# olof3/QuantumOptimalControl.jl

Measured on AMD Instinct MI355X. Metric: GRAPE gradient evals/sec (dim N, T slices, B seeds) @ 1/2/4/8 GPU, higher is better.
Workload: dtype f64

## Files before the change

quantumoptimalcontrol.jl_amd/csrc/qoc_blkseg.hpp:

```cpp
#pragma once
#include "qoc_blku.hpp"

namespace qoc {

struct BlksegParams {
  double rad[3];
  double mur[3], mui[3];
  double theta_cap;
  int S;
  int L;
  int UPW;
  int RB;
  const double* u;
  double* u_copy;
  double* u_copy2;
  double* J2;
  cx<double>* coef2;
  double* dJdu;
  unsigned long long* terms;
  unsigned int* done;
  double* best;
  long long seed_offset;
  double* best_res;
  double* best_out;
// ... 231 lines not shown
        for (int kk = 0; kk < NB; ++kk) {
          double sr = 0.0, si = 0.0;
#pragma unroll
          for (int q = 0; q < NB; ++q) {
            sr = fma(Rr[i * NB + q], xr_[q * NB + kk], fma(-Ri[i * NB + q], xi_[q * NB + kk], sr));
            si = fma(Rr[i * NB + q], xi_[q * NB + kk], fma(Ri[i * NB + q], xr_[q * NB + kk], si));
          }
          tr[kk] = sr;
          ti[kk] = si;
        }
#pragma unroll
        for (int kk = 0; kk < NB; ++kk) {
          Rr[i * NB + kk] = tr[kk];
          Ri[i * NB + kk] = ti[kk];
        }
      }
#pragma unroll
      for (int kk = 0; kk < NB; ++kk) {
        double tr[NB], ti[NB];
#pragma unroll
        for (int i = 0; i < NB; ++i) {
          double sr = Rr[i * NB + kk], si = Ri[i * NB + kk];
#pragma unroll
          for (int q = 0; q < NB; ++q) {
            sr = fma(xr_[i * NB + q], Lr[q * NB + kk], fma(-xi_[i * NB + q], Li[q * NB + kk], sr));
            si = fma(xr_[i * NB + q], Li[q * NB + kk], fma(xi_[i * NB + q], Lr[q * NB + kk], si));
          }
          tr[i] = sr;
          ti[i] = si;
        }
#pragma unroll
        for (int i = 0; i < NB; ++i) {
          Lr[i * NB + kk] = tr[i];
          Li[i * NB + kk] = ti[i];
          if constexpr (MACC) {
            Mr[i * NB + kk] = fma(invf[n + 1], tr[i], Mr[i * NB + kk]);
            Mi[i * NB + kk] = fma(invf[n + 1], ti[i], Mi[i * NB + kk]);
          }
        }
      }
      if constexpr (!MACC) seg_trace<NB>(gen, Lr, Li, invf[n + 1], m1r, m1i, m2r, m2i, acc1, acc2);
    }
  }
  if constexpr (MACC) seg_trace<NB>(gen, Mr, Mi, 1.0, m1r, m1i, m2r, m2i, acc1, acc2);
}

struct Sk2 {
  double d0, d1, r, q;
};
__device__ __forceinline__ Sk2 sk2_of(const double2 (&e)[4]) { return Sk2{e[0].y, e[3].y, e[1].x, e[1].y}; }

template <int K = BLKSEG_KMAX>
__device__ __forceinline__ void sk2_phase(double d0, double d1, double& ct, double& st) {
  constexpr BlksegTrig T = blkseg_trig();
  const double t = 0.5 * (d0 + d1), t2 = t * t;
  ct = T.c[K];
  st = T.s[K];
#pragma unroll
  for (int k = K - 1; k >= 0; --k) {
    ct = fma(ct, t2, T.c[k]);
    st = fma(st, t2, T.s[k]);
  }
  st *= t;
}
template <int K = BLKSEG_KMAX>
__device__ __forceinline__ void sk2_z(const Sk2& g0, const double* rec, double& zr, double& zi) {
  double ct, st;
  sk2_phase<K>(g0.d0, g0.d1, ct, st);
  const double2 ph = *reinterpret_cast<const double2*>(rec);
  zr = ph.x * ct - ph.y * st;
  zi = fma(ph.x, st, ph.y * ct);
}
template <int K = BLKSEG_KMAX, bool EX = false>
__device__ __forceinline__ void sk2_form(const Sk2 (&g)[3], double2 ph, double2 u, Sk2& ah, double (&ur)[4],
                                         double (&ui)[4], double* ex = nullptr) {
  constexpr BlksegTrig T = blkseg_trig();
  ah.d0 = fma(u.y, g[2].d0, fma(u.x, g[1].d0, g[0].d0));
  ah.d1 = fma(u.y, g[2].d1, fma(u.x, g[1].d1, g[0].d1));
  ah.r = fma(u.y, g[2].r, fma(u.x, g[1].r, g[0].r));
  ah.q = fma(u.y, g[2].q, fma(u.x, g[1].q, g[0].q));
  const double a = 0.5 * (ah.d0 - ah.d1);
  const double w = fma(a, a, fma(ah.r, ah.r, ah.q * ah.q));
  double cw = T.c[K], sw = T.s[K], s3 = EX ? T.d[K] : 0.0, ct, st;
#pragma unroll
  for (int k = K - 1; k >= 0; --k) {
    cw = fma(cw, w, T.c[k]);
    sw = fma(sw, w, T.s[k]);
    if constexpr (EX) s3 = fma(s3, w, T.d[k]);
  }
  sk2_phase<K>(ah.d0, ah.d1, ct, st);
  const double zr = ph.x * ct - ph.y * st, zi = fma(ph.x, st, ph.y * ct);
  const double cr = zr * cw, ci = zi * cw, sr = zr * sw, si = zi * sw;
  if constexpr (EX) {
    ex[0] = cw;
    ex[1] = sw;
    ex[2] = s3;
    ex[3] = zr;
    ex[4] = zi;
  }
  ur[0] = fma(-si, a, cr);
  ui[0] = fma(sr, a, ci);
  ur[3] = fma(si, a, cr);
  ui[3] = fma(-sr, a, ci);
  ur[1] = fma(sr, ah.r, -si * ah.q);
  ui[1] = fma(sr, ah.q, si * ah.r);
  ur[2] = fma(-sr, ah.r, -si * ah.q);
  ui[2] = fma(sr, ah.q, -si * ah.r);
}
template <int K = BLKSEG_KMAX, bool EX = false>
__device__ __forceinline__ void sk2_form_v(const Sk2 (&g)[3], double2 u, double a0, Sk2& ah, double (&v)[4],
                                           double zr = 1.0, double zi = 0.0, double* ex = nullptr) {
  constexpr BlksegTrig T = blkseg_trig();
  ah.d0 = g[0].d0;
  ah.d1 = g[0].d1;
  ah.r = fma(u.y, g[2].r, fma(u.x, g[1].r, g[0].r));
  ah.q = fma(u.y, g[2].q, fma(u.x, g[1].q, g[0].q));
  const double w = fma(a0, a0, fma(ah.r, ah.r, ah.q * ah.q));
  double cw = T.c[K], sw = T.s[K], s3 = EX ? T.d[K] : 0.0;
#pragma unroll
  for (int k = K - 1; k >= 0; --k) {
    cw = fma(cw, w, T.c[k]);
    sw = fma(sw, w, T.s[k]);
    if constexpr (EX) s3 = fma(s3, w, T.d[k]);
  }
  if constexpr (EX) {
    ex[0] = cw;
    ex[1] = sw;
    ex[2] = s3;
    ex[3] = zr;
    ex[4] = zi;
  }
  v[0] = cw;
  v[1] = sw * a0;
  v[2] = sw * ah.r;
  v[3] = sw * ah.q;
}
__device__ __forceinline__ void sk2_expand(const double (&v)[4], double (&mr)[4], double (&mi)[4]) {
  mr[0] = v[0];
  mi[0] = v[1];
  mr[1] = v[2];
  mi[1] = v[3];
  mr[2] = -v[2];
  mi[2] = v[3];
  mr[3] = v[0];
  mi[3] = -v[1];
}
__device__ __forceinline__ void sk2_vmul(const double (&v)[4], const double (&p)[4], double (&t)[4]) {
  t[0] = fma(v[0], p[0], fma(-v[1], p[1], fma(-v[2], p[2], -v[3] * p[3])));
  t[1] = fma(v[0], p[1], fma(v[1], p[0], fma(v[2], p[3], -v[3] * p[2])));
  t[2] = fma(v[0], p[2], fma(-v[1], p[3], fma(v[2], p[0], v[3] * p[1])));
  t[3] = fma(v[0], p[3], fma(v[1], p[2], fma(-v[2], p[1], v[3] * p[0])));
}

__device__ __forceinline__ void sk2_rx(double (&Rr)[4], double (&Ri)[4], const Sk2& x) {
#pragma unroll
  for (int i = 0; i < 2; ++i) {
    const double p0r = Rr[2 * i], p0i = Ri[2 * i], p1r = Rr[2 * i + 1], p1i = Ri[2 * i + 1];
    Rr[2 * i] = fma(-p0i, x.d0, fma(-p1r, x.r, -p1i * x.q));
    Ri[2 * i] = fma(p0r, x.d0, fma(p1r, x.q, -p1i * x.r));
    Rr[2 * i + 1] = fma(p0r, x.r, fma(-p0i, x.q, -p1i * x.d1));
    Ri[2 * i + 1] = fma(p0r, x.q, fma(p0i, x.r, p1r * x.d1));
  }
}
__device__ __forceinline__ void sk2_xlr(double (&Lr)[4], double (&Li)[4], const double (&Rr)[4], const double (&Ri)[4],
                                        const Sk2& x) {
#pragma unroll
  for (int k = 0; k < 2; ++k) {
    const double c0r = Lr[k], c0i = Li[k], c1r = Lr[2 + k], c1i = Li[2 + k];
    Lr[k] = fma(-x.d0, c0i, fma(x.r, c1r, fma(-x.q, c1i, Rr[k])));
    Li[k] = fma(x.d0, c0r, fma(x.r, c1i, fma(x.q, c1r, Ri[k])));
    Lr[2 + k] = fma(-x.r, c0r, fma(-x.q, c0i, fma(-x.d1, c1i, Rr[2 + k])));
    Li[2 + k] = fma(-x.r, c0i, fma(x.q, c0r, fma(x.d1, c1r, Ri[2 + k])));
  }
}
template <int ORD>
__device__ __forceinline__ void sk2_contract(const Sk2& x, const Sk2& e1, const Sk2& e2, double (&Lr)[4],
                                             double (&Li)[4], double& acc1, double& acc2) {
  constexpr double invf[6] = {1.0, 1.0, 0.5, 1.0 / 6, 1.0 / 24, 1.0 / 120};
  double Mr[4], Mi[4], Rr[4], Ri[4];
#pragma unroll
  for (int e = 0; e < 4; ++e) {
    Mr[e] = Rr[e] = Lr[e];
    Mi[e] = Ri[e] = Li[e];
  }
#pragma unroll
  for (int n = 1; n < ORD; ++n) {
    sk2_rx(Rr, Ri, x);
    sk2_xlr(Lr, Li, Rr, Ri, x);
#pragma unroll
    for (int e = 0; e < 4; ++e) {
      Mr[e] = fma(invf[n + 1], Lr[e], Mr[e]);
      Mi[e] = fma(invf[n + 1], Li[e], Mi[e]);
    }
  }
  const double dr = Mr[2] - Mr[1], di = Mi[2] + Mi[1];
  acc1 = fma(-e1.d0, Mi[0], fma(-e1.d1, Mi[3], fma(e1.r, dr, -e1.q * di)));
  acc2 = fma(-e2.d0, Mi[0], fma(-e2.d1, Mi[3], fma(e2.r, dr, -e2.q * di)));
}

template <int ORD, bool CX = false>
__device__ __forceinline__ void sk2_contract_pauli(const Sk2& x, const double (&a1)[4], const double (&a2)[4],
                                                   const double (&Kr)[4], const double (&Ki)[4], double& acc1,
                                                   double& acc2, double x0c = 0.0, double x3c = 0.0,
                                                   double x02c = 0.0) {
  static_assert(ORD >= 1 && ORD <= 3, "Pauli form for orders 1..3");
  const double k0i = Ki[0] + Ki[3], k1i = Ki[1] + Ki[2], k2i = Kr[1] - Kr[2], k3i = Ki[0] - Ki[3];
  if constexpr (CX) {
    double m1, m2;
    if constexpr (ORD == 1) {
      m1 = k1i;
      m2 = k2i;
    } else {
      const double k0r = Kr[0] + Kr[3], k1r = Kr[1] + Kr[2], k2r = Ki[2] - Ki[1];
      const double x1 = x.q, x2 = x.r;
      if constexpr (ORD == 2) {
        m1 = fma(x0c, k1r, fma(k0r, x1, k1i));
        m2 = fma(x0c, k2r, fma(k0r, x2, k2i));
      } else {
        const double di = fma(x3c, k3i, fma(x2, k2i, x1 * k1i));
        const double w = fma(x3c, x3c, fma(x2, x2, x1 * x1));
        const double al1 = fma(-0.5, x02c, fma(-1.0 / 6.0, w, 1.0));
        const double c = fma(-x0c, k0i, fma(-1.0 / 3.0, di, k0r));
        m1 = fma(al1, k1i, fma(x0c, k1r, c * x1));
        m2 = fma(al1, k2i, fma(x0c, k2r, c * x2));
      }
    }
    acc1 = fma(a1[2], m2, a1[1] * m1);
    acc2 = fma(a2[2], m2, a2[1] * m1);
    return;
  }
  double m0, m1, m2, m3;
  if constexpr (ORD == 1) {
    m0 = k0i;
    m1 = k1i;
    m2 = k2i;
    m3 = k3i;
  } else {
    const double k0r = Kr[0] + Kr[3], k1r = Kr[1] + Kr[2], k2r = Ki[2] - Ki[1], k3r = Kr[0] - Kr[3];
    const double x0 = CX ? x0c : 0.5 * (x.d0 + x.d1), x1 = x.q, x2 = x.r, x3 = CX ? x3c : 0.5 * (x.d0 - x.d1);
    const double dr = fma(x3, k3r, fma(x2, k2r, x1 * k1r)), di = fma(x3, k3i, fma(x2, k2i, x1 * k1i));
    if constexpr (ORD == 2) {
      m0 = fma(x0, k0r, k0i + dr);
      m1 = fma(x0, k1r, fma(k0r, x1, k1i));
      m2 = fma(x0, k2r, fma(k0r, x2, k2i));
      m3 = fma(x0, k3r, fma(k0r, x3, k3i));
    } else {
      const double w = fma(x3, x3, fma(x2, x2, x1 * x1)), x02 = CX ? x02c : x0 * x0;
      const double al0 = fma(-0.5, x02 + w, 1.0), al1 = fma(-0.5, x02, fma(-1.0 / 6.0, w, 1.0));
      m0 = fma(al0, k0i, fma(x0, k0r - di, dr));
      const double c = fma(-x0, k0i, fma(-1.0 / 3.0, di, k0r));
      m1 = fma(al1, k1i, fma(x0, k1r, c * x1));
      m2 = fma(al1, k2i, fma(x0, k2r, c * x2));
      m3 = fma(al1, k3i, fma(x0, k3r, c * x3));
    }
  }
  acc1 = fma(a1[3], m3, fma(a1[2], m2, fma(a1[1], m1, a1[0] * m0)));
  acc2 = fma(a2[3], m3, fma(a2[2], m2, fma(a2[1], m1, a2[0] * m0)));
}
__device__ __forceinline__ void sk2_pauli2(const Sk2& e, double (&a)[4]) {
  a[0] = -0.5 * (e.d0 + e.d1);
  a[1] = -0.5 * (2.0 * e.q);
  a[2] = -0.5 * (2.0 * e.r);
  a[3] = -0.5 * (e.d0 - e.d1);
}

template <bool CX = false>
__device__ __forceinline__ void sk2_contract_exact(const Sk2& x, const double (&a1)[4], const double (&a2)[4],
                                                   const double (&Kr)[4], const double (&Ki)[4], const double (&ex)[5],
                                                   double& acc1, double& acc2, double x3c = 0.0) {
  const double cw = ex[0], sw = ex[1], s3 = ex[2], zr = ex[3], zi = ex[4];
  const double k0i = Ki[0] + Ki[3], k1i = Ki[1] + Ki[2], k2i = Kr[1] - Kr[2], k3i = Ki[0] - Ki[3];
  const double k0r = Kr[0] + Kr[3], k1r = Kr[1] + Kr[2], k2r = Ki[2] - Ki[1], k3r = Kr[0] - Kr[3];
  const double x1 = x.q, x2 = x.r, x3 = CX ? x3c : 0.5 * (x.d0 - x.d1);
  const double dr = fma(x3, k3r, fma(x2, k2r, x1 * k1r)), di = fma(x3, k3i, fma(x2, k2i, x1 * k1i));
  const double cr = -fma(sw, k0i, s3 * dr), ci = fma(sw, k0r, -s3 * di);
  const double m1 = fma(zr, fma(sw, k1i, ci * x1), zi * fma(sw, k1r, cr * x1));
  const double m2 = fma(zr, fma(sw, k2i, ci * x2), zi * fma(sw, k2r, cr * x2));
  if constexpr (CX) {
    acc1 = fma(a1[2], m2, a1[1] * m1);
    acc2 = fma(a2[2], m2, a2[1] * m1);
  } else {
    const double n0r = fma(cw, k0r, -sw * di), n0i = fma(cw, k0i, sw * dr);
    const double m0 = fma(zr, n0i, zi * n0r);
    const double m3 = fma(zr, fma(sw, k3i, ci * x3), zi * fma(sw, k3r, cr * x3));
    acc1 = fma(a1[3], m3, fma(a1[2], m2, fma(a1[1], m1, a1[0] * m0)));
    acc2 = fma(a2[3], m3, fma(a2[2], m2, fma(a2[1], m1, a2[0] * m0)));
  }
}

template <int NB>
__device__ __forceinline__ void seg_rx(double (&Rr)[NB * NB], double (&Ri)[NB * NB], const double (&xr_)[NB * NB],
                                       const double (&xi_)[NB * NB]) {
#pragma unroll
  for (int i = 0; i < NB; ++i) {
    double tr[NB], ti[NB];
#pragma unroll
    for (int kk = 0; kk < NB; ++kk) {
      double sr = 0.0, si = 0.0;
#pragma unroll
      for (int q = 0; q < NB; ++q) {
        sr = fma(Rr[i * NB + q], xr_[q * NB + kk], fma(-Ri[i * NB + q], xi_[q * NB + kk], sr));
        si = fma(Rr[i * NB + q], xi_[q * NB + kk], fma(Ri[i * NB + q], xr_[q * NB + kk], si));
      }
      tr[kk] = sr;
      ti[kk] = si;
    }
#pragma unroll
    for (int kk = 0; kk < NB; ++kk) {
      Rr[i * NB + kk] = tr[kk];
      Ri[i * NB + kk] = ti[kk];
    }
  }
}
template <int NB>
__device__ __forceinline__ void seg_xlr(double (&Lr)[NB * NB], double (&Li)[NB * NB], const double (&Rr)[NB * NB],
                                        const double (&Ri)[NB * NB], const double (&xr_)[NB * NB],
                                        const double (&xi_)[NB * NB]) {
#pragma unroll
  for (int kk = 0; kk < NB; ++kk) {
    double tr[NB], ti[NB];
#pragma unroll
    for (int i = 0; i < NB; ++i) {
      double sr = Rr[i * NB + kk], si = Ri[i * NB + kk];
#pragma unroll
      for (int q = 0; q < NB; ++q) {
        sr = fma(xr_[i * NB + q], Lr[q * NB + kk], fma(-xi_[i * NB + q], Li[q * NB + kk], sr));
        si = fma(xr_[i * NB + q], Li[q * NB + kk], fma(xi_[i * NB + q], Lr[q * NB + kk], si));
      }
      tr[i] = sr;
      ti[i] = si;
    }
#pragma unroll
    for (int i = 0; i < NB; ++i) {
      Lr[i * NB + kk] = tr[i];
      Li[i * NB + kk] = ti[i];
    }
  }
}
template <int NB, typename GENF>
__device__ __forceinline__ void seg_contract_exact(GENF&& genf, const double (&xr_)[NB * NB], const double (&xi_)[NB * NB],
                                                   double (&Lr)[NB * NB], double (&Li)[NB * NB], int nex, double er,
                                                   double ei, double m1r, double m1i, double m2r, double m2i,
                                                   double& acc1, double& acc2) {
  constexpr int E = NB * NB;
  double Rr[E], Ri[E];
#pragma unroll
  for (int e = 0; e < E; ++e) {
    const double vr = Lr[e], vi = Li[e];
    Lr[e] = Rr[e] = er * vr - ei * vi;
    Li[e] = Ri[e] = fma(er, vi, ei * vr);
  }
  acc1 = acc2 = 0.0;
  seg_trace<NB>(genf(), Lr, Li, 1.0, m1r, m1i, m2r, m2i, acc1, acc2);
  double f = 1.0;
#pragma unroll 1
  for (int n = 1; n < nex; ++n) {
    seg_rx<NB>(Rr, Ri, xr_, xi_);
    seg_xlr<NB>(Lr, Li, Rr, Ri, xr_, xi_);
    f /= (double)(n + 1);
    seg_trace<NB>(genf(), Lr, Li, f, m1r, m1i, m2r, m2i, acc1, acc2);
  }
}

__device__ __forceinline__ double block_max(double v, double* scratch) {
  for (int off = 32; off > 0; off >>= 1) v = fmax(v, __shfl_xor(v, off));
  const int w = threadIdx.x >> 6, l = threadIdx.x & 63;
  __syncthreads();
  if (l == 0) scratch[w] = v;
  __syncthreads();
  double s = scratch[0];
  const int nw = (blockDim.x + 63) >> 6;
  for (int i = 1; i < nw; ++i) s = fmax(s, scratch[i]);
  __syncthreads();
  return s;
}

__device__ __forceinline__ void wave_lds_sync() {
  __builtin_amdgcn_fence(__ATOMIC_RELEASE, "wavefront");
  __builtin_amdgcn_wave_barrier();
  __builtin_amdgcn_fence(__ATOMIC_ACQUIRE, "wavefront");
}
// ... 813 lines not shown
        }
        seg_mm<NB, false, false>(qr, qi, dr, di, tr, ti);
#pragma unroll
        for (int i = 0; i < NB; ++i)
#pragma unroll
          for (int j = 0; j < NB; ++j) {
            double sr = 0.0, si = 0.0;
#pragma unroll
            for (int q = 0; q < NB; ++q) {
              sr = fma(tr[i * NB + q], qr[j * NB + q], fma(ti[i * NB + q], qi[j * NB + q], sr));
              si = fma(ti[i * NB + q], qr[j * NB + q], fma(-tr[i * NB + q], qi[j * NB + q], si));
            }
            if constexpr (MODE == BLKSEG_FWD) dseg_at(i * NB + j) = make_double2(sr, si);
            else dl_at(i * NB + j) = make_double2(sr, si);
          }
        __builtin_amdgcn_sched_barrier(0);
        const double f = 2.0 * sp.pen_mu;
#pragma unroll
        for (int i = 0; i < NB; ++i)
#pragma unroll
          for (int j = 0; j < NB; ++j) {
            double sr = 0.0, si = 0.0;
#pragma unroll
            for (int q = 0; q < NB; ++q) {
              sr = fma(dr[i * NB + q], Hr[q * NB + j], fma(-di[i * NB + q], Hi[q * NB + j], sr));
              si = fma(dr[i * NB + q], Hi[q * NB + j], fma(di[i * NB + q], Hr[q * NB + j], si));
            }
            hr[i * NB + j] = fma(f, sr, hr[i * NB + j]);
            hi[i * NB + j] = fma(f, si, hi[i * NB + j]);
          }
        __builtin_amdgcn_sched_barrier(0);
      }
    }
    seg_mm<NB, false, false>(qr, qi, hr, hi, tr, ti);
    seg_mm<NB, false, true>(tr, ti, qr, qi, Gr, Gi);
  }

  if (!early) publish();
  BK_T(t2e);
  BK_ADD(2, t2e - t2);
  if constexpr (MODE == BLKSEG_FWD) {
    if (sact)
#pragma unroll
      for (int e = 0; e < E; ++e) gseg_at(e) = make_double2(Gr[e], Gi[e]);
    if (sp.terms && tid == 0) atomicAdd(sp.terms + b % TERM_SLOTS, (unsigned long long)Nt * ((unsigned long long)P << J));
    return;
  }
  }
  BK_T(t3);
  const double mu1r = sp.mur[1], mu1i = sp.mui[1], mu2r = sp.mur[2], mu2i = sp.mui[2];
  const double pen2 = PEN ? 2.0 * sp.pen_mu : 0.0;
  auto pen_step = [&](const double (&ur)[E], const double (&ui)[E]) {
    seg_pen_step<NB>(pm, pen2, slot + (size_t)opaque(s) * E * nblk + beta, nblk, ur, ui, Gr, Gi);
  };
  double zr, zi;
  lane_z(zr, zi);
  if (su) {
#pragma unroll
    for (int e = 0; e < E; ++e) {
      const double t = fma(zr, Gr[e], zi * Gi[e]);
      Gi[e] = fma(zr, Gi[e], -zi * Gr[e]);
      Gr[e] = t;
    }
  }
  const double pen2r = pen2 * zr, pen2i = -pen2 * zi;
  auto pen_step_v = [&](const double (&ur)[E], const double (&ui)[E]) {
    seg_pen_step<NB, true>(pm, pen2r, slot + (size_t)opaque(s) * E * nblk + beta, nblk, ur, ui, Gr, Gi, pen2i);
  };
  double* const wr = wred + 128 * RB * w;
  const int nrl = sp.UPW * max(nu, 1);
  const int rq = l / nrl, rrem = l - rq * nrl, ro = rrem / max(nu, 1), rj = rrem - ro * max(nu, 1);
  int rslot = 0;
  auto reduce = [&](int jj, double acc1, double acc2) {
    const int r = rslot;
    rslot = r == RB - 1 ? 0 : r + 1;
    *reinterpret_cast<double2*>(wr + 128 * r + 2 * l) = make_double2(acc1, acc2);
    if (r == RB - 1 || jj == 0) {
      wave_lds_sync();
      if (rq <= r) {
        const int ss = w * sp.UPW + ro, kk = ss * L + jj + r - rq;
        if (ss < S && kk < Nt) {
          const double* src = wr + 128 * rq + 2 * ro * nblk + rj;
          double sum = 0.0;
          for (int q = 0; q < nblk; ++q) sum += src[2 * q];
          dJ[(size_t)kk * nu + rj] = sum;
        }
      }
      wave_lds_sync();
    }
  };
  double pa1[4] = {0, 0, 0, 0}, pa2[4] = {0, 0, 0, 0};
  const double zxd0 = NB == 2 ? gk[0].d0 + sp.mui[0] : 0.0, zxd1 = NB == 2 ? gk[0].d1 + sp.mui[0] : 0.0;
  const double zx0 = 0.5 * (zxd0 + zxd1), zx3 = 0.5 * (zxd0 - zxd1), zx02 = zx0 * zx0;
  if constexpr (NB == 2) {
    sk2_pauli2(Sk2{gk[1].d0 + mu1i, gk[1].d1 + mu1i, gk[1].r, gk[1].q}, pa1);
    sk2_pauli2(Sk2{gk[2].d0 + mu2i, gk[2].d1 + mu2i, gk[2].r, gk[2].q}, pa2);
  }
  double tsr = 0.0, tsi = 0.0;
  auto p3_fast = [&](int jj, auto SEL_, auto K_, auto ZD_, const double2* upre = nullptr) {
    constexpr bool SEL = decltype(SEL_)::value;
    constexpr int KS = decltype(K_)::value;
    constexpr bool ZD = decltype(ZD_)::value;
    if constexpr (NB == 2) {
      const int k = kb + jj;
      const bool act = !SEL || (sact && k < ke);
      const double* r = SEL ? rec + 4 * (size_t)(act ? k : 0) : reck + 4 * (size_t)jj;
      const double2 u = upre ? *upre : *reinterpret_cast<const double2*>(r + 2);
      Sk2 ah;
      double ur[4], ui[4], ex[5];
      if constexpr (ZD) {
        double vv[4];
        sk2_form_v<KS, ORD == 0>(gk, u, za0, ah, vv, zr, zi, ex);
        sk2_expand(vv, ur, ui);
      } else {
        sk2_form<KS, ORD == 0>(gk, *reinterpret_cast<const double2*>(r), u, ah, ur, ui, ex);
      }
      if constexpr (PEN) {
        if (pm && (!SEL || act)) {
          if constexpr (ZD) pen_step_v(ur, ui);
          else pen_step(ur, ui);
        }
      }
      double Kr[4], Ki[4], tr[4], ti[4];
      seg_mm<2, true, false>(ur, ui, Gr, Gi, Kr, Ki);
      seg_mm<2, false, false>(Kr, Ki, ur, ui, tr, ti);
#pragma unroll
      for (int e = 0; e < 4; ++e) {
        Gr[e] = !SEL || act ? tr[e] : Gr[e];
        Gi[e] = !SEL || act ? ti[e] : Gi[e];
      }
      const double mki = ZD ? sp.mui[0] : fma(u.y, mu2i, fma(u.x, mu1i, sp.mui[0]));
      const Sk2 x{ah.d0 + mki, ah.d1 + mki, ah.r, ah.q};
      if constexpr (TS) {
        const double t_re = fma(-x.d0, ti[0], fma(-x.d1, ti[3], fma(x.r, tr[2] - tr[1], -x.q * (ti[2] + ti[1]))));
        tsr += !SEL || act ? t_re : 0.0;
        if constexpr (ZD) {
          const double t_im = fma(x.d0, tr[0], fma(x.d1, tr[3], fma(x.r, ti[2] - ti[1], x.q * (tr[2] + tr[1]))));
          tsi += !SEL || act ? t_im : 0.0;
        }
      }
      double acc1, acc2;
      if constexpr (ORD == 0) {
        sk2_contract_exact<ZD>(x, pa1, pa2, Kr, Ki, ex, acc1, acc2, zx3);
      } else if constexpr (ORD <= 3) {
        sk2_contract_pauli<ORD, ZD>(x, pa1, pa2, Kr, Ki, acc1, acc2, zx0, zx3, zx02);
      } else {
        const Sk2 e1{gk[1].d0 + mu1i, gk[1].d1 + mu1i, gk[1].r, gk[1].q};
        const Sk2 e2{gk[2].d0 + mu2i, gk[2].d1 + mu2i, gk[2].r, gk[2].q};
        sk2_contract<ORD>(x, e1, e2, Kr, Ki, acc1, acc2);
      }
      reduce(jj, !SEL || act ? acc1 : 0.0, !SEL || act ? acc2 : 0.0);
    }
  };
  auto loop3z = [&](auto K_, auto ZD_) {
    int jj = L - 1;
    for (; jj >= Lf; --jj) {
      if (turns) seg_turn(grp, ngrp, jj);
      sprog.step(L + (L - 1 - jj));
      p3_fast(jj, std::true_type(), K_, ZD_);
    }
    constexpr bool PRE = decltype(ZD_)::value;
    double2 un = make_double2(0.0, 0.0);
    if (PRE && jj >= 0) un = *reinterpret_cast<const double2*>(reck + 4 * (size_t)jj + 2);
    for (; jj >= 0; --jj) {
      if (turns) seg_turn(grp, ngrp, jj);
      sprog.step(L + (L - 1 - jj));
      const double2 uc = un;
      if constexpr (PRE) {
        un = *reinterpret_cast<const double2*>(reck + 4 * (size_t)max(jj - 1, 0) + 2);
        __builtin_amdgcn_sched_barrier(0);
      }
      p3_fast(jj, std::false_type(), K_, ZD_, PRE ? &uc : nullptr);
    }
  };
  auto loop3 = [&](auto K_) {
    if (zd) loop3z(K_, std::true_type());
    else loop3z(K_, std::false_type());
  };
  if (fast) {
    if (ksel == 5) loop3(std::integral_constant<int, 5>());
    else if (ksel == 7) loop3(std::integral_constant<int, 7>());
    else loop3(std::integral_constant<int, BLKSEG_KMAX>());
  } else {
    for (int jj = L - 1; jj >= 0; --jj) {
      if (turns) seg_turn(grp, ngrp, jj);
      sprog.step(L + (L - 1 - jj));
      const int k = kb + jj;
      const bool act = sact && k < ke;
      const double* rk[1] = {rec + 4 * (size_t)(act ? k : 0)};
      const auto gen = gen_at(GREG ? beta : opaque(beta));
      double ar[1][E], ai[1][E], ur[1][E], ui[1][E];
      seg_form<NB, 1>(gen, rk, s0, P, J, ar, ai, ur, ui);
      if constexpr (PEN) {
        if (pm && act) pen_step(ur[0], ui[0]);
      }
      constexpr bool TSE = TS && NB == 3 && ORD == 1;
      if constexpr (TSE) {
        double t_re = 0.0, gtr = 0.0, gti = 0.0;
#pragma unroll
        for (int i = 0; i < NB; ++i) {
          gtr += Gr[i * NB + i];
          gti += Gi[i * NB + i];
#pragma unroll
          for (int q = 0; q < NB; ++q)
            t_re = fma(ar[0][i * NB + q], Gr[q * NB + i], fma(-ai[0][i * NB + q], Gi[q * NB + i], t_re));
        }
        const double2 sv = *reinterpret_cast<const double2*>(rk[0] + 2);
        const double v1 = ldexp(sv.x, J), v2 = ldexp(sv.y, J);
        const double nr = fma(v2, sp.mur[2], fma(v1, sp.mur[1], sp.mur[0]));
        const double ni = fma(v2, sp.mui[2], fma(v1, sp.mui[1], sp.mui[0]));
        t_re = fma(nr, gtr, fma(-ni, gti, ldexp(t_re, J)));
        tsr += act ? t_re : 0.0;
      }
      double Kr[E], Ki[E], tr[E], ti[E];
      seg_mm<NB, true, false>(ur[0], ui[0], Gr, Gi, Kr, Ki);
      seg_mm<NB, false, false>(Kr, Ki, ur[0], ui[0], tr, ti);
#pragma unroll
      for (int e = 0; e < E; ++e) {
        Gr[e] = act ? tr[e] : Gr[e];
        Gi[e] = act ? ti[e] : Gi[e];
      }
      const double2 su = *reinterpret_cast<const double2*>(rk[0] + 2);
      const double u1 = ldexp(su.x, J), u2 = ldexp(su.y, J);
      const double mkr = fma(u2, sp.mur[2], fma(u1, sp.mur[1], sp.mur[0]));
      const double mki = fma(u2, sp.mui[2], fma(u1, sp.mui[1], sp.mui[0]));
      const double dgr = ORD == 0 ? 0.0 : mkr, dgi = ORD == 0 ? 0.0 : mki;
      double xr[E], xi[E];
      if constexpr (XA) {
#pragma unroll
        for (int e = 0; e < E; ++e) {
          xr[e] = (J ? ldexp(ar[0][e], J) : ar[0][e]) + (e % (NB + 1) == 0 ? dgr : 0.0);
          xi[e] = (J ? ldexp(ai[0][e], J) : ai[0][e]) + (e % (NB + 1) == 0 ? dgi : 0.0);
        }
      } else {
        const auto gen2 = gen_at(opaque(beta));
#pragma unroll
        for (int e = 0; e < E; ++e) {
          const double2 g0 = gen2(0, e), g1 = gen2(1, e), g2 = gen2(2, e);
          xr[e] = fma(u2, g2.x, fma(u1, g1.x, g0.x)) + (e % (NB + 1) == 0 ? dgr : 0.0);
          xi[e] = fma(u2, g2.y, fma(u1, g1.y, g0.y)) + (e % (NB + 1) == 0 ? dgi : 0.0);
        }
      }
      if constexpr (TS && !TSE) {
        double t_re = 0.0;
#pragma unroll
        for (int i = 0; i < NB; ++i)
#pragma unroll
          for (int q = 0; q < NB; ++q)
            t_re = fma(xr[i * NB + q], Gr[q * NB + i], fma(-xi[i * NB + q], Gi[q * NB + i], t_re));
        if constexpr (ORD == 0) {
          double gtr = 0.0, gti = 0.0;
#pragma unroll
          for (int i = 0; i < NB; ++i) {
            gtr += Gr[i * NB + i];
            gti += Gi[i * NB + i];
          }
          t_re = fma(mkr, gtr, fma(-mki, gti, t_re));
        }
        tsr += act ? t_re : 0.0;
      }
      double acc1, acc2;
      constexpr bool GST = ORD == 0 && NB == 3 && !PEN;
      if constexpr (GST) {
        double2* const gp = slot + (size_t)opaque(sact ? s : 0) * E * nblk + beta;
        if (sact)
#pragma unroll
          for (int e = 0; e < E; ++e) gp[e * nblk] = make_double2(Gr[e], Gi[e]);
      }
      if constexpr (ORD == 0) {
        seg_contract_exact<NB>([&] { return gen_at(GREG ? beta : opaque(beta)); }, xr, xi, Kr, Ki, nex, rk[0][0],
                               rk[0][1], mu1r, mu1i, mu2r, mu2i, acc1, acc2);
      } else {
        seg_contract<NB, ORD, XA>(gen, xr, xi, Kr, Ki, mu1r, mu1i, mu2r, mu2i, acc1, acc2);
      }
      if constexpr (GST) {
        const double2* const gp = slot + (size_t)opaque(sact ? s : 0) * E * nblk + beta;
#pragma unroll
        for (int e = 0; e < E; ++e) {
          const double2 v = gp[e * nblk];
          Gr[e] = v.x;
          Gi[e] = v.y;
        }
      }
      reduce(jj, act ? acc1 : 0.0, act ? acc2 : 0.0);
    }
  }
  if (turns || sprog.on) __builtin_amdgcn_s_setprio(0);
  BK_T(t4);
  BK_ADD(3, t4 - t3);
  SEGW_SET(16 + w, t4 - t0);
  if constexpr (TS) {
    double v = su ? zr * tsr - zi * tsi : tsr;
    v = sact ? v : 0.0;
    for (int off = 32; off > 0; off >>= 1) v += __shfl_xor(v, off);
    if (l == 0) red[w] = v;
  }
  __syncthreads();
  if constexpr (TS) {
    if (tid == 0) {
      double sum = 0.0;
      for (int q = 0; q < W; ++q) sum += red[q];
      sp.dJdtau[b] = sum / tau;
    }
  }
  double* const og = sp.dJdu + (size_t)b * Nt * nu;
  for (int i = tid; i < Nt * nu; i += nthr) og[i] = dJ[i];
  if (MODE == BLKSEG_FUSED && sp.terms && tid == 0)
    atomicAdd(sp.terms + b % TERM_SLOTS, (unsigned long long)Nt * ((unsigned long long)P << J));
  BK_T(t5);
  BK_ADD(4, t5 - t4);
  BK_ADD(5, t5 - t0);
}

template <bool VEC>
__global__ __launch_bounds__(256) void k_ens_reduce(int B, int E, int n, const double* __restrict__ w,
                                                    const double* __restrict__ g, const double* __restrict__ Jm,
                                                    double* __restrict__ dJdu, double* __restrict__ J,
                                                    double* __restrict__ J2) {
  const int nv = VEC ? n / 2 : n;
  const long long idx = (long long)blockIdx.x * blockDim.x + threadIdx.x;
  if (idx < (long long)B * nv) {
    const int p = (int)(idx / nv), i = (int)(idx - (long long)p * nv);
    if constexpr (VEC) {
      const double2* src = reinterpret_cast<const double2*>(g + (size_t)p * E * n) + i;
      double2 acc = make_double2(0.0, 0.0);
// ... 154 lines not shown
```

Before: 4.757 million.

## Propagate backward costate in Pauli basis for 2x2 zero-drift third pass

Adds a Pauli-coordinate path for the backward sweep when NB==2, no penalty and expansion order 1..3. The costate is kept as eight Pauli coefficients and rotated with cross-product formulas, replacing complex 2x2 matrix products, and the contraction reuses the precomputed coefficients. It also inserts an explicit waitcnt after the first prefetch. The aim is fewer FLOPs and registers per time slice, at the cost of more template paths and possible numerical differences.

```diff
diff --git a/quantumoptimalcontrol.jl_amd/csrc/qoc_blkseg.hpp b/quantumoptimalcontrol.jl_amd/csrc/qoc_blkseg.hpp
--- a/quantumoptimalcontrol.jl_amd/csrc/qoc_blkseg.hpp
+++ b/quantumoptimalcontrol.jl_amd/csrc/qoc_blkseg.hpp
@@ -407,6 +407,54 @@
   t[3] = fma(v[0], p[3], fma(v[1], p[2], fma(-v[2], p[1], v[3] * p[0])));
 }
 
+__device__ __forceinline__ void sk2_pauli_of(const double (&mr)[4], const double (&mi)[4], double (&gp)[8]) {
+  gp[0] = mr[0] + mr[3];
+  gp[1] = mi[0] + mi[3];
+  gp[2] = mr[1] + mr[2];
+  gp[3] = mi[2] - mi[1];
+  gp[4] = mr[0] - mr[3];
+  gp[5] = mi[1] + mi[2];
+  gp[6] = mr[1] - mr[2];
+  gp[7] = mi[0] - mi[3];
+}
+template <int ORD>
+__device__ __forceinline__ void sk2_pauli_k(const double (&v)[4], const double (&gp)[8], double (&tc)[6],
+                                            double (&kc)[7]) {
+  const double v0 = v[0], n1 = v[3], n2 = v[2], n3 = v[1];
+  const double* a = gp + 1;
+  const double* b = gp + 4;
+  tc[0] = fma(n2, a[3], -n3 * a[2]);
+  tc[1] = fma(n3, a[1], -n1 * a[3]);
+  tc[2] = fma(n1, a[2], -n2 * a[1]);
+  tc[3] = fma(n2, b[3], -n3 * b[2]);
+  tc[4] = fma(n3, b[1], -n1 * b[3]);
+  tc[5] = fma(n1, b[2], -n2 * b[1]);
+  kc[3] = fma(v0, b[1], fma(-gp[0], n1, tc[3]));
+  kc[5] = fma(v0, b[2], fma(-gp[0], n2, tc[4]));
+  if constexpr (ORD >= 2) {
+    const double di = fma(n3, b[3], fma(n2, b[2], n1 * b[1]));
+    kc[0] = fma(v0, gp[0], di);
+    kc[2] = fma(v0, a[1], fma(gp[1], n1, tc[0]));
+    kc[4] = fma(v0, a[2], fma(gp[1], n2, tc[1]));
+  }
+  if constexpr (ORD >= 3) {
+    const double dr = fma(n3, a[3], fma(n2, a[2], n1 * a[1]));
+    kc[1] = fma(v0, gp[1], -dr);
+    kc[6] = fma(v0, b[3], fma(-gp[0], n3, tc[5]));
+  }
+}
+__device__ __forceinline__ void sk2_pauli_rot(const double (&v)[4], const double (&tc)[6], const double (&gp)[8],
+                                              double (&gn)[6]) {
+  const double w0 = 2.0 * v[0], m1 = 2.0 * v[3], m2 = 2.0 * v[2], m3 = 2.0 * v[1];
+#pragma unroll
+  for (int c = 0; c < 2; ++c) {
+    const double t1 = tc[3 * c], t2 = tc[3 * c + 1], t3 = tc[3 * c + 2];
+    gn[3 * c] = fma(m2, t3, fma(-m3, t2, fma(w0, t1, gp[2 + 3 * c])));
+    gn[3 * c + 1] = fma(m3, t1, fma(-m1, t3, fma(w0, t2, gp[3 + 3 * c])));
+    gn[3 * c + 2] = fma(m1, t2, fma(-m2, t1, fma(w0, t3, gp[4 + 3 * c])));
+  }
+}
+
 __device__ __forceinline__ void sk2_rx(double (&Rr)[4], double (&Ri)[4], const Sk2& x) {
 #pragma unroll
   for (int i = 0; i < 2; ++i) {
@@ -453,6 +501,34 @@
   acc2 = fma(-e2.d0, Mi[0], fma(-e2.d1, Mi[3], fma(e2.r, dr, -e2.q * di)));
 }
 
+template <int ORD>
+__device__ __forceinline__ void sk2_contract_pauli_k(double x1, double x2, const double (&a1)[4],
+                                                     const double (&a2)[4], const double (&kc)[7], double& acc1,
+                                                     double& acc2, double x0c, double x3c, double x02c) {
+  static_assert(ORD >= 1 && ORD <= 3, "Pauli form for orders 1..3");
+  const double k1i = kc[3], k2i = kc[5];
+  double m1, m2;
+  if constexpr (ORD == 1) {
+    m1 = k1i;
+    m2 = k2i;
+  } else {
+    const double k0r = kc[0], k1r = kc[2], k2r = kc[4];
+    if constexpr (ORD == 2) {
+      m1 = fma(x0c, k1r, fma(k0r, x1, k1i));
+      m2 = fma(x0c, k2r, fma(k0r, x2, k2i));
+    } else {
+      const double k0i = kc[1], k3i = kc[6];
+      const double di = fma(x3c, k3i, fma(x2, k2i, x1 * k1i));
+      const double w = fma(x3c, x3c, fma(x2, x2, x1 * x1));
+      const double al1 = fma(-0.5, x02c, fma(-1.0 / 6.0, w, 1.0));
+      const double c = fma(-x0c, k0i, fma(-1.0 / 3.0, di, k0r));
+      m1 = fma(al1, k1i, fma(x0c, k1r, c * x1));
+      m2 = fma(al1, k2i, fma(x0c, k2r, c * x2));
+    }
+  }
+  acc1 = fma(a1[2], m2, a1[1] * m1);
+  acc2 = fma(a2[2], m2, a2[1] * m1);
+}
 template <int ORD, bool CX = false>
 __device__ __forceinline__ void sk2_contract_pauli(const Sk2& x, const double (&a1)[4], const double (&a2)[4],
                                                    const double (&Kr)[4], const double (&Ki)[4], double& acc1,
@@ -461,27 +537,13 @@
   static_assert(ORD >= 1 && ORD <= 3, "Pauli form for orders 1..3");
   const double k0i = Ki[0] + Ki[3], k1i = Ki[1] + Ki[2], k2i = Kr[1] - Kr[2], k3i = Ki[0] - Ki[3];
   if constexpr (CX) {
-    double m1, m2;
-    if constexpr (ORD == 1) {
-      m1 = k1i;
-      m2 = k2i;
-    } else {
-      const double k0r = Kr[0] + Kr[3], k1r = Kr[1] + Kr[2], k2r = Ki[2] - Ki[1];
-      const double x1 = x.q, x2 = x.r;
-      if constexpr (ORD == 2) {
-        m1 = fma(x0c, k1r, fma(k0r, x1, k1i));
-        m2 = fma(x0c, k2r, fma(k0r, x2, k2i));
-      } else {
-        const double di = fma(x3c, k3i, fma(x2, k2i, x1 * k1i));
-        const double w = fma(x3c, x3c, fma(x2, x2, x1 * x1));
-        const double al1 = fma(-0.5, x02c, fma(-1.0 / 6.0, w, 1.0));
-        const double c = fma(-x0c, k0i, fma(-1.0 / 3.0, di, k0r));
-        m1 = fma(al1, k1i, fma(x0c, k1r, c * x1));
-        m2 = fma(al1, k2i, fma(x0c, k2r, c * x2));
-      }
-    }
-    acc1 = fma(a1[2], m2, a1[1] * m1);
-    acc2 = fma(a2[2], m2, a2[1] * m1);
+    double kc[7] = {0.0, k0i, 0.0, k1i, 0.0, k2i, k3i};
+    if constexpr (ORD >= 2) {
+      kc[0] = Kr[0] + Kr[3];
+      kc[2] = Kr[1] + Kr[2];
+      kc[4] = Ki[2] - Ki[1];
+    }
+    sk2_contract_pauli_k<ORD>(x.q, x.r, a1, a2, kc, acc1, acc2, x0c, x3c, x02c);
     return;
   }
   double m0, m1, m2, m3;
@@ -1601,16 +1663,55 @@
       reduce(jj, !SEL || act ? acc1 : 0.0, !SEL || act ? acc2 : 0.0);
     }
   };
+  constexpr bool PAU = NB == 2 && !PEN && ORD >= 1 && ORD <= 3;
+  double gp[8];
+  auto p3_pauli = [&](int jj, auto SEL_, auto K_, const double2* upre = nullptr) {
+    constexpr bool SEL = decltype(SEL_)::value;
+    constexpr int KS = decltype(K_)::value;
+    if constexpr (PAU) {
+      const int k = kb + jj;
+      const bool act = !SEL || (sact && k < ke);
+      const double* r = SEL ? rec + 4 * (size_t)(act ? k : 0) : reck + 4 * (size_t)jj;
+      const double2 u = upre ? *upre : *reinterpret_cast<const double2*>(r + 2);
+      Sk2 ah;
+      double vv[4], tc[6], kc[7], gn[6];
+      sk2_form_v<KS>(gk, u, za0, ah, vv);
+      sk2_pauli_k<ORD>(vv, gp, tc, kc);
+      sk2_pauli_rot(vv, tc, gp, gn);
+#pragma unroll
+      for (int e = 0; e < 6; ++e) gp[2 + e] = !SEL || act ? gn[e] : gp[2 + e];
+      if constexpr (TS) {
+        const double t_re = -fma(ah.q, gn[3], fma(ah.r, gn[4], fma(zx3, gn[5], zx0 * gp[1])));
+        const double t_im = fma(ah.q, gn[0], fma(ah.r, gn[1], fma(zx3, gn[2], zx0 * gp[0])));
+        tsr += !SEL || act ? t_re : 0.0;
+        tsi += !SEL || act ? t_im : 0.0;
+      }
+      double acc1, acc2;
+      sk2_contract_pauli_k<ORD>(ah.q, ah.r, pa1, pa2, kc, acc1, acc2, zx0, zx3, zx02);
+      reduce(jj, !SEL || act ? acc1 : 0.0, !SEL || act ? acc2 : 0.0);
+    }
+  };
   auto loop3z = [&](auto K_, auto ZD_) {
+    constexpr bool PZ = PAU && decltype(ZD_)::value;
+    auto p3 = [&](int jj, auto SEL_, const double2* upre = nullptr) {
+      if constexpr (PZ) p3_pauli(jj, SEL_, K_, upre);
+      else p3_fast(jj, SEL_, K_, ZD_, upre);
+    };
+    if constexpr (PAU) {
+      if constexpr (PZ) sk2_pauli_of(Gr, Gi, gp);
+    }
     int jj = L - 1;
     for (; jj >= Lf; --jj) {
       if (turns) seg_turn(grp, ngrp, jj);
       sprog.step(L + (L - 1 - jj));
-      p3_fast(jj, std::true_type(), K_, ZD_);
+      p3(jj, std::true_type());
     }
     constexpr bool PRE = decltype(ZD_)::value;
     double2 un = make_double2(0.0, 0.0);
-    if (PRE && jj >= 0) un = *reinterpret_cast<const double2*>(reck + 4 * (size_t)jj + 2);
+    if (PRE && jj >= 0) {
+      un = *reinterpret_cast<const double2*>(reck + 4 * (size_t)jj + 2);
+      __builtin_amdgcn_s_waitcnt(0xc07f);
+    }
     for (; jj >= 0; --jj) {
       if (turns) seg_turn(grp, ngrp, jj);
       sprog.step(L + (L - 1 - jj));
@@ -1619,7 +1720,7 @@
         un = *reinterpret_cast<const double2*>(reck + 4 * (size_t)max(jj - 1, 0) + 2);
         __builtin_amdgcn_sched_barrier(0);
       }
-      p3_fast(jj, std::false_type(), K_, ZD_, PRE ? &uc : nullptr);
+      p3(jj, std::false_type(), PRE ? &uc : nullptr);
     }
   };
   auto loop3 = [&](auto K_) {
```

New measurement: 4.980 million, median of 6. 1.05x the previous value.
